# weentiaan/Video-latent-diffusion-panoptic-segmentation

Hardware: NVIDIA B200
Metric: panoptic frames/sec (DDIM-50, 384x1248 KITTI) (higher is better)
Workload: dtype bf16

## Files before the change

video_latent_diffusion_panoptic_segmentation_b200/csrc/gemm_tc.cu:

```cuda
#include <stdlib.h>
#include <string.h>

#include "gemm_tc_kernel.cuh"

namespace ldm_gemm {
#define LDM_GEMM_DECLARE(NAME)                                                                                      \
  cudaError_t NAME(bool pair, int grid, int smem_bytes, cudaStream_t stream, const CUtensorMap& tmA1,               \
                   const CUtensorMap& tmA2, const CUtensorMap& tmB, const CUtensorMap& tmO, const CUtensorMap& tmR, \
                   const CUtensorMap& tmE, const GemmParams& p);
LDM_GEMM_DECLARE(launch_gemm_staged)
LDM_GEMM_DECLARE(launch_gemm_geglu)
LDM_GEMM_DECLARE(launch_gemm_qkv)
LDM_GEMM_DECLARE(launch_gemm_direct)
LDM_GEMM_DECLARE(launch_gemm_convt)
LDM_GEMM_DECLARE(launch_gemm_split)
LDM_GEMM_DECLARE(launch_gemm_geglu_ln)
LDM_GEMM_DECLARE(launch_gemm_qkv_ln)
}

namespace {

using namespace ldm;
using namespace ldm_gemm;

void pick_box(int H, int W, int taps, int* bw_out, int* bh_out) {
  (void)taps;
  if (H == 1) {
    *bw_out = W < 128 ? W : 128;
    *bh_out = 1;
    return;
  }
  long best_tiles = -1;
  int best_bw = 1, best_bh = 1;
  for (int bw = 1; bw <= 128 && bw <= W; ++bw) {
    int bh = 128 / bw;
    if (bh > H) bh = H;
    if (bh < 1) continue;
    const long tiles = (long)((W + bw - 1) / bw) * ((H + bh - 1) / bh);
    if (best_tiles < 0 || tiles < best_tiles || (tiles == best_tiles && bw > best_bw)) {
      best_tiles = tiles;
      best_bw = bw;
      best_bh = bh;
    }
  }
  *bw_out = best_bw;
  *bh_out = best_bh;
}

int pick_block_n(int N, long m_tiles, long kblocks, int sms, bool pair, int taps, double* cost_out, int max_split = 1,
                 long ws_floats = 0, int* split_out = nullptr) {
  static const int cands[] = {256, 224, 192, 160, 128, 96};
  static const double mma_single[] = {167, 158, 151, 141, 111, 106};
  static const double mma_pair[] = {160, 149, 136, 124, 99, 92};
  static const int splits[] = {1, 2, 3, 4, 5, 6, 8, 10, 12, 16};
  int best = 256, best_s = 256, best_split = 1;
  double best_cost = -1.0, best_cost_s = -1.0;
  const long m_units = pair ? (m_tiles + 1) / 2 : m_tiles;
  const long m_alloc = pair ? 2 * m_units : m_units;
  const long workers = pair ? sms / 2 : sms;
  for (int i = 0; i < 6; ++i) {
    const int c = cands[i];
    if (c == 224 && taps != 9) continue;
    const long n_tiles = (N + c - 1) / c;
    for (int si = 0; si < 10; ++si) {
      const int sp = splits[si];
      if (sp > max_split) break;
      if (sp > 1) {
        if (kblocks / sp < (pair ? 24 : 8)) break;
        if ((long)sp * m_alloc * n_tiles * c * 128 > ws_floats) break;
      }
      const long waves = (m_units * n_tiles * sp + workers - 1) / workers;
      const double item = (double)((kblocks + sp - 1) / sp) * 4.0 * (pair ? mma_pair[i] : mma_single[i]) +
                          (pair ? 3300.0 + 11.0 * c : 1000.0 + 17.0 * c) + (sp > 1 ? 8.0 * c : 0.0);
      double cost = (double)waves * item;
      if (sp > 1) cost += 6000.0 + (double)sp * m_alloc * n_tiles * c * 128.0 * 4.0 / 2000.0;
      if (sp == 1) {
        if (best_cost < 0 || cost < best_cost * 0.999) {
          best_cost = cost;
          best = c;
        }
      } else if (best_cost_s < 0 || cost < best_cost_s * 0.999) {
        best_cost_s = cost;
        best_s = c;
        best_split = sp;
      }
    }
  }
  if (best_cost_s > 0 && best_cost_s < 0.88 * best_cost) {
    best_cost = best_cost_s;
    best = best_s;
  } else {
    best_split = 1;
  }
  if (cost_out) *cost_out = best_cost;
  if (split_out) *split_out = best_split;
  return best;
}

int debug_flags() {
  using ldm_host::diag_env_has;
  int v = 0;
  if (diag_env_has("LDM_GEMM_DEBUG", "notma")) v |= kDbgNoTma;
  if (diag_env_has("LDM_GEMM_DEBUG", "nomma")) v |= kDbgNoMma;
  if (diag_env_has("LDM_GEMM_DEBUG", "nowait")) v |= kDbgNoWait | kDbgNoTma;
  if (diag_env_has("LDM_GEMM_DEBUG", "nofence")) v |= kDbgNoFence;
  if (diag_env_has("LDM_GEMM_DEBUG", "keepcommit")) v |= kDbgKeepCommit;
  return v;
}

int resmma_max_kblocks() { return ldm_host::diag_env("LDM_GEMM_RESMMA", 1 << 30); }

bool staged_enabled() { return ldm_host::diag_env("LDM_GEMM_STAGED", 1) != 0; }

bool splitk_enabled() { return ldm_host::diag_env("LDM_GEMM_SPLITK", 1) != 0; }

thread_local int g_last_cfg[3] = {0, 0, 1};

constexpr size_t kSplitCounterBytes = 0;

struct FixupParams {
  const float* ws;
  long long slice_stride;
  int split, tiles_x, tiles_y, bw, bh, W, H, m_tiles, n_tiles, block_n, N, silu;
  const float* bias;
  const float* rowbias;
  const __nv_bfloat16* residual;
  __nv_bfloat16* out;
};

__global__ void __launch_bounds__(256) splitk_fixup_kernel(const FixupParams p) {
  __shared__ float tile[kBlockM][17];
  pdl_launch_dependents();
  pdl_wait();
  const int cb = blockIdx.x, n_tile = blockIdx.y, m_tile = blockIdx.z;
  const int warp = threadIdx.x >> 5, lane = threadIdx.x & 31;
  const long long tile_off = ((long long)m_tile * p.n_tiles + n_tile) * (long long)(p.block_n * kBlockM);
  {
    float a[8];
#pragma unroll
    for (int k = 0; k < 8; ++k) a[k] = 0.f;
    const float* src = p.ws + tile_off + (long long)(cb * 16 + warp * 2) * kBlockM + lane;
    for (int s0 = 0; s0 < p.split; s0 += 4) {
      float v[4][8];
#pragma unroll
      for (int q = 0; q < 4; ++q)
#pragma unroll
        for (int k = 0; k < 8; ++k)
          v[q][k] = s0 + q < p.split ? __ldcg(src + (long long)(s0 + q) * p.slice_stride + (k >> 2) * kBlockM + (k & 3) * 32) : 0.f;
#pragma unroll
      for (int q = 0; q < 4; ++q)
#pragma unroll
        for (int k = 0; k < 8; ++k) a[k] += v[q][k];
    }
#pragma unroll
    for (int k = 0; k < 8; ++k) tile[(k & 3) * 32 + lane][warp * 2 + (k >> 2)] = a[k];
  }
  __syncthreads();
  const int r = threadIdx.x >> 1, vec = threadIdx.x & 1;
  const int tiles_per_img = p.tiles_x * p.tiles_y;
  const int b = m_tile / tiles_per_img;
  const int rem = m_tile - b * tiles_per_img;
  const int ty = rem / p.tiles_x, tx = rem - ty * p.tiles_x;
  const int ly = r / p.bw, lx = r - ly * p.bw;
  const int y = ty * p.bh + ly, x = tx * p.bw + lx;
  const int n = n_tile * p.block_n + cb * 16 + vec * 8;
  if (r >= p.bw * p.bh || y >= p.H || x >= p.W || n >= p.N) return;
  const long long grow = ((long long)b * p.H + y) * p.W + x;
  float f[8];
#pragma unroll
  for (int j = 0; j < 8; ++j) f[j] = tile[r][vec * 8 + j];
  if (p.bias) {
    const float4 b0 = __ldg(reinterpret_cast<const float4*>(p.bias + n)), b1 = __ldg(reinterpret_cast<const float4*>(p.bias + n + 4));
    f[0] += b0.x; f[1] += b0.y; f[2] += b0.z; f[3] += b0.w; f[4] += b1.x; f[5] += b1.y; f[6] += b1.z; f[7] += b1.w;
  }
  if (p.rowbias) {
    const float* rb = p.rowbias + (long long)b * p.N + n;
    const float4 b0 = __ldg(reinterpret_cast<const float4*>(rb)), b1 = __ldg(reinterpret_cast<const float4*>(rb + 4));
    f[0] += b0.x; f[1] += b0.y; f[2] += b0.z; f[3] += b0.w; f[4] += b1.x; f[5] += b1.y; f[6] += b1.z; f[7] += b1.w;
  }
  if (p.residual) {
    const uint4 u = ld_nc_v4(p.residual + grow * p.N + n);
    const float2 a0 = unpack_bf16(u.x), a1 = unpack_bf16(u.y), a2 = unpack_bf16(u.z), a3 = unpack_bf16(u.w);
    f[0] += a0.x; f[1] += a0.y; f[2] += a1.x; f[3] += a1.y; f[4] += a2.x; f[5] += a2.y; f[6] += a3.x; f[7] += a3.y;
  }
  if (p.silu) {
#pragma unroll
    for (int j = 0; j < 8; ++j) f[j] = silu_f(f[j]);
  }
  store_bf16x8(p.out + grow * p.N + n, f);
// ... 325 lines not shown
```

video_latent_diffusion_panoptic_segmentation_b200/csrc/gemm_tc_kernel.cuh:

```cuda
#pragma once
#include "common.cuh"
#include "host_util.h"

namespace ldm_gemm {

using namespace ldm;

constexpr int kBlockM = 128;
constexpr int kBlockK = 64;
constexpr int kABytes = kBlockM * kBlockK * 2;
constexpr int kMaxStages = 8;
constexpr int kEpiWarps = 8;
constexpr int kThreads = 64 + 32 * kEpiWarps;
constexpr int kSmemBudget = 227 * 1024;
constexpr int kEpiStageBytes = 2 * 16384 + 1280;
constexpr int kStagedStore = 1 << 20;
constexpr int kQkvStaged = 1 << 21;
constexpr int kDbgNoTma = 1 << 29;
constexpr int kDbgNoMma = 1 << 30;
constexpr int kDbgNoFence = 1 << 27;
constexpr int kDbgKeepCommit = 1 << 26;
constexpr int kDbgNoWait = 1 << 28;

struct GemmParams {
  int tiles_x, tiles_y, B, bw, bh, W, H;
  int m_tiles, n_tiles, block_n;
  int N, taps, kblocks1, kblocks, ktap;
  int stages, stage_bytes;
  int res_kblocks;
  int flags;
  const float* bias;
  const float* rowbias;
  const __nv_bfloat16* residual;
  void* out;
  __nv_bfloat16* q;
  __nv_bfloat16* k;
  __nv_bfloat16* vt;
  const float* ln_gamma;
  const float* ln_beta;
  float ln_eps;
  int heads, head_dim, dpad, seq, seq_pad, vt_rows;
  int qkv_part0;
  unsigned long long magic_seq, magic_c, magic_d;
  int a_stride;
  int a_pad;
  int up2_ntiles;
  int up2_cout;
  int n_store;
  long long img_px;
  float* row_stats;
  const float* ln_stats;
  const float* ln_colsum;
  int ln_parts;
  long long rows_total;
  float ln_invc, ln_fold_eps;
  int split_k;
  float* ws;
  long long ws_slice_stride;
};

__device__ __forceinline__ void store_bf16x8(__nv_bfloat16* dst, const float* v) {
  uint4 u;
  u.x = pack_bf16(v[0], v[1]);
  u.y = pack_bf16(v[2], v[3]);
  u.z = pack_bf16(v[4], v[5]);
  u.w = pack_bf16(v[6], v[7]);
  *reinterpret_cast<uint4*>(dst) = u;
}

enum { kEpiStaged = 0, kEpiGeglu = 1, kEpiQkv = 2, kEpiDirect = 3, kEpiConvT = 4, kEpiSplit = 5, kEpiGegluLn = 6, kEpiQkvLn = 7 };

template <bool kPair, int kEpiT>
__global__ void __launch_bounds__(kThreads, 1)
gemm_tc_kernel(const __grid_constant__ CUtensorMap tmA1, const __grid_constant__ CUtensorMap tmA2,
               const __grid_constant__ CUtensorMap tmB, const __grid_constant__ CUtensorMap tmO,
               const __grid_constant__ CUtensorMap tmR, const __grid_constant__ CUtensorMap tmE, const GemmParams p) {
  constexpr bool kLn = kEpiT == kEpiGegluLn || kEpiT == kEpiQkvLn;
  constexpr int kEpi = kEpiT == kEpiGegluLn ? (int)kEpiGeglu : kEpiT == kEpiQkvLn ? (int)kEpiQkv : kEpiT;
  extern __shared__ __align__(1024) uint8_t smem_raw[];
  uint8_t* smem = smem_raw + ((1024u - (smem_u32(smem_raw) & 1023u)) & 1023u);
  uint8_t* epi_smem = smem + p.stages * p.stage_bytes;
  uint64_t* full_bar = reinterpret_cast<uint64_t*>(epi_smem + kEpiStageBytes);
  uint64_t* empty_bar = full_bar + kMaxStages;
  uint64_t* tfull_bar = empty_bar + kMaxStages;
  uint64_t* tempty_bar = tfull_bar + 2;
  uint32_t* tmem_slot = reinterpret_cast<uint32_t*>(tempty_bar + 2);

  const int warp = __shfl_sync(0xffffffffu, (int)(threadIdx.x >> 5), 0);
  const int lane = threadIdx.x & 31;
  const uint32_t rank = kPair ? cluster_ctarank() : 0u;
  const int worker = kPair ? (int)(blockIdx.x >> 1) : (int)blockIdx.x;
  const int num_workers = kPair ? (int)(gridDim.x >> 1) : (int)gridDim.x;

  if (warp == 0 && lane == 0) {
    tma_prefetch_desc(&tmA1);
    tma_prefetch_desc(&tmA2);
    tma_prefetch_desc(&tmB);
    tma_prefetch_desc(&tmO);
    for (int i = 0; i < p.stages; ++i) {
      mbar_init(&full_bar[i], 1);
      mbar_init(&empty_bar[i], 1);
    }
    for (int i = 0; i < 2; ++i) {
      mbar_init(&tfull_bar[i], 1);
      mbar_init(&tempty_bar[i], (kPair ? 2 : 1) * kEpiWarps);
    }
    mbar_fence_init();
  }
  if (warp == 1) {
    if (kPair) {
      tmem_alloc_pair(tmem_slot, 512);
      tmem_relinquish_pair();
    } else {
      tmem_alloc(tmem_slot, 512);
      tmem_relinquish();
    }
  }
  tc_fence_before();
  if (kPair) cluster_sync_all(); else __syncthreads();
  tc_fence_after();
  const uint32_t tmem_base = *tmem_slot;
  pdl_launch_dependents();
  pdl_wait();

  const int m_units = kPair ? (p.m_tiles + 1) / 2 : p.m_tiles;
  const int num_tiles = m_units * p.n_tiles;
  constexpr bool kSplit = kEpi == kEpiSplit;
  const int split = kSplit ? p.split_k : 1;
  const int num_items = num_tiles * split;
  const int kmain = p.taps * p.kblocks;
  const int tiles_per_img = p.tiles_x * p.tiles_y;
  const uint32_t a_bytes = (uint32_t)(p.bw * p.bh) * (kBlockK * 2);
  const int b_rows = kPair ? p.block_n / 2 : p.block_n;
  const uint32_t b_bytes = (uint32_t)b_rows * (kBlockK * 2);

  if (warp == 0) {
    {
      int stage = 0;
      uint32_t phase = 0;
      for (int item = worker; item < num_items; item += num_workers) {
        const int tile = kSplit ? item / split : item;
        const int slice = kSplit ? item - tile * split : 0;
        const int k_lo = kSplit ? (int)((long long)kmain * slice / split) : 0;
        const int k_hi = kSplit ? (int)((long long)kmain * (slice + 1) / split) : kmain;
        const int n_tile = tile / m_units;
        const int m_unit = tile - n_tile * m_units;
        const int m_tile = kPair ? 2 * m_unit + (int)rank : m_unit;
        const int b = m_tile / tiles_per_img;
        const int rem = m_tile - b * tiles_per_img;
        const int ty = rem / p.tiles_x;
        const int tx = rem - ty * p.tiles_x;
        const int x0 = tx * p.bw, y0 = ty * p.bh;
        const int n0 = n_tile * p.block_n + (int)rank * b_rows;
        int tap = k_lo / p.kblocks, kb = k_lo - tap * p.kblocks;
        const int cls = p.up2_ntiles > 0 ? n_tile / p.up2_ntiles : 0;
        const int ax0 = x0 * p.a_stride, ay0 = y0 * p.a_stride;
        for (int ki = k_lo; ki < k_hi; ++ki) {
          const int dy = (p.taps == 9) ? tap / 3 - p.a_pad : (p.taps == 4) ? (tap >> 1) - 1 + (cls >> 1) : 0;
          const int dx = (p.taps == 9) ? tap % 3 - p.a_pad : (p.taps == 4) ? (tap & 1) - 1 + (cls & 1) : 0;
          {
            if (p.flags & kDbgNoWait) continue;
            mbar_wait(&empty_bar[stage], phase ^ 1);
            uint8_t* sa = smem + stage * p.stage_bytes;
            uint8_t* sb = sa + kABytes;
            const CUtensorMap* tmA = (kb < p.kblocks1) ? &tmA1 : &tmA2;
            const int kc = (kb < p.kblocks1 ? kb : kb - p.kblocks1) * kBlockK;
            if (!elect_one()) {
            } else if (p.flags & kDbgNoTma) {
              if (rank == 0) mbar_arrive(&full_bar[stage]);
            } else if (kPair) {
              if (rank == 0) mbar_arrive_expect_tx(&full_bar[stage], 2 * (a_bytes + b_bytes));
              tma_load_4d_pair(sa, tmA, &full_bar[stage], kc, ax0 + dx, ay0 + dy, b);
              tma_load_2d_pair(sb, &tmB, &full_bar[stage], tap * p.ktap + kb * kBlockK, n0);
            } else {
              mbar_arrive_expect_tx(&full_bar[stage], a_bytes + b_bytes);
              tma_load_4d(sa, tmA, &full_bar[stage], kc, ax0 + dx, ay0 + dy, b);
              tma_load_2d(sb, &tmB, &full_bar[stage], tap * p.ktap + kb * kBlockK, n0);
            }
            if (++stage == p.stages) {
              stage = 0;
              phase ^= 1;
            }
          }
          if (++kb == p.kblocks) {
            kb = 0;
            ++tap;
          }
        }
        const int nres = (slice == split - 1) ? p.res_kblocks : 0;
        for (int j = 0; j < nres; ++j) {
          mbar_wait(&empty_bar[stage], phase ^ 1);
          uint8_t* sa = smem + stage * p.stage_bytes;
          uint8_t* sb = sa + kABytes;
          if (elect_one()) {
            if (kPair) {
              if (rank == 0) mbar_arrive_expect_tx(&full_bar[stage], 2 * (a_bytes + b_bytes));
              tma_load_4d_pair(sa, &tmR, &full_bar[stage], n_tile * p.block_n + j * kBlockK, x0, y0, b);
              tma_load_2d_pair(sb, &tmE, &full_bar[stage], j * kBlockK, (int)rank * b_rows);
            } else {
              mbar_arrive_expect_tx(&full_bar[stage], a_bytes + b_bytes);
              tma_load_4d(sa, &tmR, &full_bar[stage], n_tile * p.block_n + j * kBlockK, x0, y0, b);
              tma_load_2d(sb, &tmE, &full_bar[stage], j * kBlockK, 0);
            }
          }
          if (++stage == p.stages) {
            stage = 0;
            phase ^= 1;
          }
        }
      }
    }
    __syncwarp();
  } else if (warp == 1) {
    if (rank == 0) {
      const uint32_t idesc = umma_idesc_bf16(kPair ? 256 : kBlockM, (uint32_t)p.block_n);
      int stage = 0;
      uint32_t phase = 0;
      int as = 0;
      uint32_t aphase = 0;
      for (int item = worker; item < num_items; item += num_workers) {
        int ksteps = kmain + p.res_kblocks;
        if (kSplit) {
          const int slice = item % split;
          ksteps = (int)((long long)kmain * (slice + 1) / split) - (int)((long long)kmain * slice / split) +
                   (slice == split - 1 ? p.res_kblocks : 0);
        }
        mbar_wait(&tempty_bar[as], aphase ^ 1);
        tc_fence_after();
        const uint32_t d_tmem = tmem_base + (uint32_t)as * 256u;
        for (int ks = 0; ks < ksteps; ++ks) {
          if (!(p.flags & kDbgNoWait)) {
            mbar_wait(&full_bar[stage], phase);
            if (!(p.flags & kDbgNoFence)) tc_fence_after();
          }
          const uint32_t sa = smem_u32(smem + stage * p.stage_bytes);
          const uint64_t da = umma_desc_k_sw128(sa);
          const uint64_t db = umma_desc_k_sw128(sa + kABytes);
          if (elect_one()) {
#pragma unroll
            for (int k = 0; k < kBlockK / 16; ++k) {
              if (p.flags & kDbgNoMma) break;
              const uint32_t dt = d_tmem;
              if (kPair)
                umma_bf16_pair(dt, da + (uint64_t)(2 * k), db + (uint64_t)(2 * k), idesc, (ks | k) != 0);
              else
                umma_bf16(dt, da + (uint64_t)(2 * k), db + (uint64_t)(2 * k), idesc, (ks | k) != 0);
            }
            if ((p.flags & kDbgNoWait) && !(p.flags & kDbgKeepCommit)) {
            } else if (kPair) umma_commit_pair(&empty_bar[stage]); else umma_commit(&empty_bar[stage]);
          }
          __syncwarp();
          if (++stage == p.stages) {
            stage = 0;
            phase ^= 1;
          }
        }
        if (elect_one()) {
          if (kPair) umma_commit_pair(&tfull_bar[as]); else umma_commit(&tfull_bar[as]);
        }
        __syncwarp();
        if (++as == 2) {
          as = 0;
          aphase ^= 1;
        }
      }
    }
    __syncwarp();
  } else {
    const int quad = warp & 3;
    const int half = (warp - 2) >> 2;
    const int r = quad * 32 + lane;
    constexpr bool geglu = kEpi == kEpiGeglu;
    constexpr bool staged = kEpi == kEpiStaged || kEpi == kEpiGeglu;
    const bool plain = kEpi == kEpiStaged || (kEpi == kEpiDirect && !(p.flags & LDM_GEMM_GEGLU));
    const bool epi_leader = threadIdx.x == 64;
    int sb = 0;
    int as = 0;
    uint32_t aphase = 0;
    constexpr int kLnPre = 20;
    [[maybe_unused]] float2 ln_pre[kLnPre];
    [[maybe_unused]] auto ln_issue = [&](int item2) {
      const int tile2 = kSplit ? item2 / split : item2;
      const int n_tile2 = tile2 / m_units;
      const int m_unit2 = tile2 - n_tile2 * m_units;
      const int m_tile2 = kPair ? 2 * m_unit2 + (int)rank : m_unit2;
      const int b2 = m_tile2 / tiles_per_img;
      const int rem2 = m_tile2 - b2 * tiles_per_img;
      const int ty2 = rem2 / p.tiles_x;
      const int tx2 = rem2 - ty2 * p.tiles_x;
      const int ly2 = r / p.bw, lx2 = r - ly2 * p.bw;
      const int y2 = ty2 * p.bh + ly2, x2 = tx2 * p.bw + lx2;
      const bool valid2 = (m_tile2 < p.m_tiles) && (r < p.bw * p.bh) && (y2 < p.H) && (x2 < p.W);
      const float2* sp = reinterpret_cast<const float2*>(p.ln_stats) + (((long long)b2 * p.H + y2) * p.W + x2);
#pragma unroll
      for (int j = 0; j < kLnPre; ++j)
        ln_pre[j] = (valid2 && j < p.ln_parts) ? __ldg(sp + (long long)j * p.rows_total) : make_float2(0.f, 0.f);
    };
    if constexpr (kLn) {
      if (worker < num_items) ln_issue(worker);
    }
    for (int item = worker; item < num_items; item += num_workers) {
      const int tile = kSplit ? item / split : item;
      const int slice = kSplit ? item - tile * split : 0;
      const int n_tile = tile / m_units;
      const int m_unit = tile - n_tile * m_units;
      const int m_tile = kPair ? 2 * m_unit + (int)rank : m_unit;
      const int b = m_tile / tiles_per_img;
      const int rem = m_tile - b * tiles_per_img;
      const int ty = rem / p.tiles_x;
      const int tx = rem - ty * p.tiles_x;
      const int ly = r / p.bw, lx = r - ly * p.bw;
      const int y = ty * p.bh + ly, x = tx * p.bw + lx;
      const bool valid = (m_tile < p.m_tiles) && (r < p.bw * p.bh) && (y < p.H) && (x < p.W);
      const long long grow = ((long long)b * p.H + y) * p.W + x;
      const int n0 = n_tile * p.block_n;
      int qkv_bi = 0, qkv_s = 0;
      const bool qkv_vec = kEpi == kEpiQkv && (p.seq % 8 == 0) && p.bh == 1 && p.bw == kBlockM;
      if (kEpi == kEpiQkv) {
        qkv_bi = (int)(((unsigned long long)grow * p.magic_seq) >> 40);
        qkv_s = (int)(grow - (long long)qkv_bi * p.seq);
      }

      float ln_a = 1.f, ln_c = 0.f;
      constexpr bool ln_fold = kLn;
      if constexpr (ln_fold) {
        float su = 0.f, sq = 0.f;
#pragma unroll
        for (int j = 0; j < kLnPre; ++j) {
          su += ln_pre[j].x;
          sq += ln_pre[j].y;
        }
        if (valid) {
          const float2* sp = reinterpret_cast<const float2*>(p.ln_stats) + grow;
          for (int i = kLnPre; i < p.ln_parts; i += 10) {
            float2 t[10];
#pragma unroll
            for (int j = 0; j < 10; ++j)
              t[j] = i + j < p.ln_parts ? __ldg(sp + (long long)(i + j) * p.rows_total) : make_float2(0.f, 0.f);
#pragma unroll
            for (int j = 0; j < 10; ++j) {
              su += t[j].x;
              sq += t[j].y;
            }
          }
        }
        const float mean = su * p.ln_invc;
        ln_a = rsqrtf(fmaxf(fmaf(-mean, mean, sq * p.ln_invc), 0.f) + p.ln_fold_eps);
        ln_c = -mean * ln_a;
        if (item + num_workers < num_items) ln_issue(item + num_workers);
      }
      const bool ln_smem = kEpi == kEpiQkv && ln_fold && p.block_n <= 160;
      float* sLn = reinterpret_cast<float*>(epi_smem + 2 * 16384);
      if (ln_smem) {
        named_bar_sync(1, 32 * kEpiWarps);
        const int t = threadIdx.x - 64;
        if (t < p.block_n) {
          const int n = n0 + t;
          sLn[t] = (p.bias && n < p.N) ? __ldg(p.bias + n) : 0.f;
          sLn[160 + t] = n < p.N ? __ldg(p.ln_colsum + n) : 0.f;
        }
        named_bar_sync(1, 32 * kEpiWarps);
      }
      uint4 rs[4][4];
      const bool use_res = !kSplit && plain && p.residual != nullptr && valid && p.res_kblocks == 0;
      if (use_res) {
        const __nv_bfloat16* rrow = p.residual + grow * p.N + n0;
#pragma unroll
        for (int ci = 0; ci < 4; ++ci) {
          const int c = staged ? (ci * 64 < p.block_n ? min(ci * 64, p.block_n - 64) + half * 32 : p.block_n)
                               : (2 * ci + half) * 32;
#pragma unroll
          for (int g = 0; g < 4; ++g)
            if (c < p.block_n && n0 + c + g * 8 < p.N) rs[ci][g] = ld_nc_v4(rrow + c + g * 8);
        }
      }

      constexpr bool tile_bias = staged && !kSplit && !kLn;
      if constexpr (tile_bias) {
        float* sbias = reinterpret_cast<float*>(epi_smem + 2 * 16384);
        const int t = threadIdx.x - 64;
        if (t < p.block_n) {
          const int n = n0 + t;
          float bv = 0.f;
          if (n < p.N) {
            if (p.bias) bv = __ldg(p.bias + n);
            if (p.rowbias) bv += __ldg(p.rowbias + (long long)b * p.N + n);
          }
          sbias[t] = bv;
        }
      }
      mbar_wait(&tfull_bar[as], aphase);
      tc_fence_after();
      const uint32_t t_addr = tmem_base + ((uint32_t)(quad * 32) << 16) + (uint32_t)as * 256u;

      if constexpr (kSplit) {
        const long long tile_off = ((long long)m_tile * p.n_tiles + n_tile) * (long long)(p.block_n * kBlockM);
        float* wdst = p.ws + (long long)slice * p.ws_slice_stride + tile_off + r;
        for (int c = half * 32; c < p.block_n; c += 64) {
          uint32_t v[32];
          tmem_ld32(t_addr + c, v);
          tmem_ld_wait();
#pragma unroll
          for (int j = 0; j < 32; ++j) wdst[(c + j) * kBlockM] = __uint_as_float(v[j]);
        }
      }

      if constexpr (kSplit) {
      } else if constexpr (kEpi == kEpiConvT) {
        if (half == 0) {
        const int cout = p.block_n;
        float mean = 0.f;
        for (int c = 0; c < cout; c += 32) {
          uint32_t v[32];
          tmem_ld32(t_addr + c, v);
          tmem_ld_wait();
#pragma unroll
          for (int j = 0; j < 32; ++j) mean += __uint_as_float(v[j]) + __ldg(&p.bias[n0 + c + j]);
        }
        mean /= (float)cout;
        float var = 0.f;
        for (int c = 0; c < cout; c += 32) {
          uint32_t v[32];
          tmem_ld32(t_addr + c, v);
          tmem_ld_wait();
#pragma unroll
          for (int j = 0; j < 32; ++j) {
            const float d = __uint_as_float(v[j]) + __ldg(&p.bias[n0 + c + j]) - mean;
            var += d * d;
          }
        }
        const float rstd = 1.0f / sqrtf(var / (float)cout + p.ln_eps);
        const int sub = n_tile;
        const long long orow = ((long long)b * (2 * p.H) + (2 * y + (sub >> 1))) * (2 * p.W) + (2 * x + (sub & 1));
        __nv_bfloat16* dst = reinterpret_cast<__nv_bfloat16*>(p.out) + orow * cout;
        for (int c = 0; c < cout; c += 32) {
          uint32_t v[32];
          tmem_ld32(t_addr + c, v);
          tmem_ld_wait();
          if (valid) {
#pragma unroll
            for (int g = 0; g < 4; ++g) {
              float o[8];
#pragma unroll
              for (int j = 0; j < 8; ++j) {
                const int cc = c + g * 8 + j;
                const float xn = (__uint_as_float(v[g * 8 + j]) + __ldg(&p.bias[n0 + cc]) - mean) * rstd;
                o[j] = silu_f(__ldg(&p.ln_gamma[cc]) * xn + __ldg(&p.ln_beta[cc]));
              }
              store_bf16x8(dst + c + g * 8, o);
            }
          }
        }
        }
      } else if constexpr (staged) {
        const int acc_w = geglu ? 128 : 64;
#pragma unroll
        for (int ob = 0; ob < 4; ++ob) {
          if (ob * acc_w >= p.block_n) break;
          const int c0 = min(ob * acc_w, p.block_n - acc_w);
          uint8_t* sbuf = epi_smem + sb * 16384;
          float* sbias = reinterpret_cast<float*>(epi_smem + 2 * 16384);
          float* sgsum = sbias + 128;
          if (epi_leader) bulk_wait_read1();
          if constexpr (!tile_bias) {
            const int t = threadIdx.x - 64;
            if (t < acc_w) {
              const int n = n0 + c0 + t;
              float bv = 0.f;
              if (n < p.N) {
                if (p.bias) bv = __ldg(p.bias + n);
                if (p.rowbias) bv += __ldg(p.rowbias + (long long)b * p.N + n);
              }
              sbias[t] = bv;
              if (ln_fold) sgsum[t] = n < p.N ? __ldg(p.ln_colsum + n) : 0.f;
            }
          }
          named_bar_sync(1, 32 * kEpiWarps);
          uint8_t* rowp = sbuf + r * 128;
#pragma unroll
          for (int cq = 0; cq < 2; ++cq) {
            if (!geglu && cq == 1) break;
            const int cc = geglu ? half * 64 + cq * 32 : half * 32;
            const int c = c0 + cc;
            uint32_t v[32];
            tmem_ld32(t_addr + c, v);
            const int nc = n0 + c;
            float f[32];
            {
              const float4* bp = reinterpret_cast<const float4*>(sbias + (tile_bias ? c : cc));
              if (ln_fold) {
                tmem_ld_wait();
                const float4* gp = reinterpret_cast<const float4*>(sgsum + cc);
#pragma unroll
                for (int g = 0; g < 8; ++g) {
                  const float4 bv = bp[g], gv = gp[g];
                  f[g * 4] = fmaf(ln_a, __uint_as_float(v[g * 4]), fmaf(ln_c, gv.x, bv.x));
                  f[g * 4 + 1] = fmaf(ln_a, __uint_as_float(v[g * 4 + 1]), fmaf(ln_c, gv.y, bv.y));
                  f[g * 4 + 2] = fmaf(ln_a, __uint_as_float(v[g * 4 + 2]), fmaf(ln_c, gv.z, bv.z));
                  f[g * 4 + 3] = fmaf(ln_a, __uint_as_float(v[g * 4 + 3]), fmaf(ln_c, gv.w, bv.w));
                }
              } else {
                float4 bv[8];
#pragma unroll
                for (int g = 0; g < 8; ++g) bv[g] = bp[g];
                tmem_ld_wait();
#pragma unroll
                for (int g = 0; g < 8; ++g) {
                  f[g * 4] = __uint_as_float(v[g * 4]) + bv[g].x;
                  f[g * 4 + 1] = __uint_as_float(v[g * 4 + 1]) + bv[g].y;
                  f[g * 4 + 2] = __uint_as_float(v[g * 4 + 2]) + bv[g].z;
                  f[g * 4 + 3] = __uint_as_float(v[g * 4 + 3]) + bv[g].w;
                }
              }
            }
            if (geglu) {
              float o[16];
#pragma unroll
              for (int j = 0; j < 16; ++j) o[j] = f[j] * gelu_erf_fast(f[16 + j]);
#pragma unroll
              for (int g = 0; g < 2; ++g) {
                uint4 u;
                u.x = pack_bf16(o[g * 8 + 0], o[g * 8 + 1]); u.y = pack_bf16(o[g * 8 + 2], o[g * 8 + 3]);
                u.z = pack_bf16(o[g * 8 + 4], o[g * 8 + 5]); u.w = pack_bf16(o[g * 8 + 6], o[g * 8 + 7]);
                *reinterpret_cast<uint4*>(rowp + ((((cc >> 5) * 2 + g) ^ (r & 7)) << 4)) = u;
              }
            } else {
              if (use_res) {
#pragma unroll
                for (int g = 0; g < 4; ++g) {
                  if (nc + g * 8 >= p.N) break;
                  const uint4 u = rs[ob][g];
                  const float2 a0 = unpack_bf16(u.x), a1 = unpack_bf16(u.y), a2 = unpack_bf16(u.z), a3 = unpack_bf16(u.w);
                  f[g * 8 + 0] += a0.x; f[g * 8 + 1] += a0.y; f[g * 8 + 2] += a1.x; f[g * 8 + 3] += a1.y;
                  f[g * 8 + 4] += a2.x; f[g * 8 + 5] += a2.y; f[g * 8 + 6] += a3.x; f[g * 8 + 7] += a3.y;
                }
              }
              if (p.flags & LDM_GEMM_SILU) {
#pragma unroll
                for (int j = 0; j < 32; ++j) f[j] = silu_f(f[j]);
              }
              float st_s = 0.f, st_q = 0.f;
#pragma unroll
              for (int g = 0; g < 4; ++g) {
                uint4 u;
                u.x = pack_bf16(f[g * 8 + 0], f[g * 8 + 1]); u.y = pack_bf16(f[g * 8 + 2], f[g * 8 + 3]);
                u.z = pack_bf16(f[g * 8 + 4], f[g * 8 + 5]); u.w = pack_bf16(f[g * 8 + 6], f[g * 8 + 7]);
                *reinterpret_cast<uint4*>(rowp + (((half * 4 + g) ^ (r & 7)) << 4)) = u;
                if (kEpi == kEpiStaged && p.row_stats) {
                  const float2 a0 = unpack_bf16(u.x), a1 = unpack_bf16(u.y), a2 = unpack_bf16(u.z), a3 = unpack_bf16(u.w);
                  st_s += ((a0.x + a0.y) + (a1.x + a1.y)) + ((a2.x + a2.y) + (a3.x + a3.y));
                  st_q = fmaf(a0.x, a0.x, st_q); st_q = fmaf(a0.y, a0.y, st_q); st_q = fmaf(a1.x, a1.x, st_q);
                  st_q = fmaf(a1.y, a1.y, st_q); st_q = fmaf(a2.x, a2.x, st_q); st_q = fmaf(a2.y, a2.y, st_q);
                  st_q = fmaf(a3.x, a3.x, st_q); st_q = fmaf(a3.y, a3.y, st_q);
                }
              }
              if (kEpi == kEpiStaged && p.row_stats && valid && nc < p.N)
                *reinterpret_cast<float2*>(p.row_stats + ((long long)(nc >> 5) * p.rows_total + grow) * 2) =
                    make_float2(st_s, st_q);
            }
          }
          fence_proxy_async_smem();
          named_bar_sync(1, 32 * kEpiWarps);
          if (epi_leader) {
            if (p.up2_ntiles > 0) {
              const int cls = n_tile / p.up2_ntiles;
              tma_store_4d(&tmO, sbuf, n0 + c0 - cls * p.up2_cout, 2 * tx * p.bw + (cls & 1), 2 * ty * p.bh + (cls >> 1), b);
            } else {
              const int ncol = geglu ? (n0 + c0) / 2 : n0 + c0;
              tma_store_4d(&tmO, sbuf, ncol, tx * p.bw, ty * p.bh, b);
            }
            bulk_commit();
          }
          sb ^= 1;
        }
      } else {
        bool qkv_done = false;
        if constexpr (kEpi == kEpiQkv) {
          const int C = p.heads * p.head_dim;
          const int part_in = n0 / C;
          const int which_t = part_in + p.qkv_part0;
          const long long grow0 = (long long)m_tile * kBlockM;
          const int bi0 = (int)(((unsigned long long)grow0 * p.magic_seq) >> 40);
          const int s0 = (int)(grow0 - (long long)bi0 * p.seq);
          const int nimg = (int)(((long long)p.W * p.H * p.B) / p.seq);
          if ((p.flags & kQkvStaged) && which_t < 2 && (s0 + kBlockM <= p.seq || bi0 + 1 >= nimg)) {
            const int head0 = (n0 - part_in * C) / p.head_dim;
            const int heads_in_tile = p.block_n / p.head_dim;
            const int blocks_per_head = p.dpad >> 6;
            for (int hd = 0; hd < heads_in_tile; ++hd) {
              for (int kb = 0; kb < blocks_per_head; ++kb) {
                uint8_t* sbuf = epi_smem + sb * 16384;
                if (epi_leader) bulk_wait_read1();
                named_bar_sync(1, 32 * kEpiWarps);
                const int cbase = hd * p.head_dim + kb * 64 + half * 32;
                int ng = ((hd + 1) * p.head_dim - cbase) >> 3;
                ng = ng < 0 ? 0 : (ng > 4 ? 4 : ng);
                uint32_t v[32];
#pragma unroll
                for (int g = 0; g < 4; ++g)
                  if (g < ng) tmem_ld8(t_addr + cbase + g * 8, v + g * 8);
                tmem_ld_wait();
                if (ln_fold) {
#pragma unroll
                  for (int g = 0; g < 4; ++g)
                    if (g < ng) {
                      const int cl = cbase + g * 8;
                      float4 g0, g1, b0, b1;
                      if (ln_smem) {
                        b0 = *reinterpret_cast<const float4*>(sLn + cl);
                        b1 = *reinterpret_cast<const float4*>(sLn + cl + 4);
                        g0 = *reinterpret_cast<const float4*>(sLn + 160 + cl);
                        g1 = *reinterpret_cast<const float4*>(sLn + 160 + cl + 4);
                      } else {
                        const int n = n0 + cl;
                        g0 = __ldg(reinterpret_cast<const float4*>(p.ln_colsum + n));
                        g1 = __ldg(reinterpret_cast<const float4*>(p.ln_colsum + n + 4));
                        b0 = make_float4(0.f, 0.f, 0.f, 0.f), b1 = b0;
                        if (p.bias) {
                          b0 = __ldg(reinterpret_cast<const float4*>(p.bias + n));
                          b1 = __ldg(reinterpret_cast<const float4*>(p.bias + n + 4));
                        }
                      }
                      const float gv[8] = {g0.x, g0.y, g0.z, g0.w, g1.x, g1.y, g1.z, g1.w};
                      const float bv[8] = {b0.x, b0.y, b0.z, b0.w, b1.x, b1.y, b1.z, b1.w};
#pragma unroll
                      for (int j = 0; j < 8; ++j)
                        v[g * 8 + j] = __float_as_uint(fmaf(ln_a, __uint_as_float(v[g * 8 + j]), fmaf(ln_c, gv[j], bv[j])));
                    }
                }
                uint8_t* rowp = sbuf + r * 128;
#pragma unroll
                for (int g = 0; g < 4; ++g) {
                  uint4 u = make_uint4(0, 0, 0, 0);
                  if (g < ng) {
                    u.x = pack_bf16(__uint_as_float(v[g * 8 + 0]), __uint_as_float(v[g * 8 + 1]));
                    u.y = pack_bf16(__uint_as_float(v[g * 8 + 2]), __uint_as_float(v[g * 8 + 3]));
                    u.z = pack_bf16(__uint_as_float(v[g * 8 + 4]), __uint_as_float(v[g * 8 + 5]));
                    u.w = pack_bf16(__uint_as_float(v[g * 8 + 6]), __uint_as_float(v[g * 8 + 7]));
                  }
                  *reinterpret_cast<uint4*>(rowp + (((half * 4 + g) ^ (r & 7)) << 4)) = u;
                }
                fence_proxy_async_smem();
                named_bar_sync(1, 32 * kEpiWarps);
                if (epi_leader) {
                  if (which_t == 0) tma_store_4d(&tmO, sbuf, kb * 64, s0, head0 + hd, bi0);
                  else tma_store_4d(&tmR, sbuf, kb * 64, s0, head0 + hd, bi0);
                  bulk_commit();
                }
                sb ^= 1;
              }
            }
            qkv_done = true;
          }
          if ((p.flags & kQkvStaged) && !qkv_done) {
            if (epi_leader) bulk_wait_read0();
            named_bar_sync(1, 32 * kEpiWarps);
          }
        }
#pragma unroll
        for (int ci = 0; ci < 4; ++ci) {
          if (qkv_done) break;
          const int c = (2 * ci + half) * 32;
          if (c >= p.block_n) break;
          uint32_t v[32];
          tmem_ld32(t_addr + c, v);
          tmem_ld_wait();
          if (!valid && kEpi != kEpiQkv) continue;
          const int nc = n0 + c;
          if (nc >= p.N) continue;
          float f[32];
#pragma unroll
          for (int j = 0; j < 32; ++j) f[j] = __uint_as_float(v[j]);
          if (ln_smem) {
            const float4* bp = reinterpret_cast<const float4*>(sLn + c);
            const float4* gp = reinterpret_cast<const float4*>(sLn + 160 + c);
#pragma unroll
            for (int g = 0; g < 8; ++g)
              if (nc + g * 4 < p.N) {
                const float4 gv = gp[g], bv = bp[g];
                f[g * 4] = fmaf(ln_a, f[g * 4], fmaf(ln_c, gv.x, bv.x));
                f[g * 4 + 1] = fmaf(ln_a, f[g * 4 + 1], fmaf(ln_c, gv.y, bv.y));
                f[g * 4 + 2] = fmaf(ln_a, f[g * 4 + 2], fmaf(ln_c, gv.z, bv.z));
                f[g * 4 + 3] = fmaf(ln_a, f[g * 4 + 3], fmaf(ln_c, gv.w, bv.w));
              }
          } else if (ln_fold) {
            const float4* gp = reinterpret_cast<const float4*>(p.ln_colsum + nc);
#pragma unroll
            for (int g = 0; g < 8; ++g)
              if (nc + g * 4 < p.N) {
                const float4 gv = __ldg(gp + g);
                f[g * 4] = fmaf(ln_a, f[g * 4], ln_c * gv.x); f[g * 4 + 1] = fmaf(ln_a, f[g * 4 + 1], ln_c * gv.y);
                f[g * 4 + 2] = fmaf(ln_a, f[g * 4 + 2], ln_c * gv.z); f[g * 4 + 3] = fmaf(ln_a, f[g * 4 + 3], ln_c * gv.w);
              }
          }
          if (p.bias && !ln_smem) {
            const float4* bp = reinterpret_cast<const float4*>(p.bias + nc);
#pragma unroll
            for (int g = 0; g < 8; ++g)
              if (nc + g * 4 < p.N) {
                const float4 bv = __ldg(bp + g);
                f[g * 4] += bv.x; f[g * 4 + 1] += bv.y; f[g * 4 + 2] += bv.z; f[g * 4 + 3] += bv.w;
              }
          }
          if (p.rowbias) {
            const float4* bp = reinterpret_cast<const float4*>(p.rowbias + (long long)b * p.N + nc);
#pragma unroll
            for (int g = 0; g < 8; ++g)
              if (nc + g * 4 < p.N) {
                const float4 bv = __ldg(bp + g);
                f[g * 4] += bv.x; f[g * 4 + 1] += bv.y; f[g * 4 + 2] += bv.z; f[g * 4 + 3] += bv.w;
              }
          }
          if (p.flags & LDM_GEMM_GEGLU) {
            float o[16];
#pragma unroll
            for (int j = 0; j < 16; ++j) o[j] = f[j] * gelu_erf_fast(f[16 + j]);
            __nv_bfloat16* dst = reinterpret_cast<__nv_bfloat16*>(p.out) + grow * (p.N / 2) + nc / 2;
            store_bf16x8(dst, o);
            store_bf16x8(dst + 8, o + 8);
            continue;
          }
          if constexpr (kEpi == kEpiQkv) {
            const int C = p.heads * p.head_dim;
#pragma unroll
            for (int g = 0; g < 4; ++g) {
              const int n = nc + g * 8;
              if (n >= p.N) break;
              const int part = (int)(((unsigned long long)(unsigned)n * p.magic_c) >> 40);
              const int cc = n - part * C;
              const int which = part + p.qkv_part0;
              const int head = (int)(((unsigned long long)(unsigned)cc * p.magic_d) >> 40);
              const int e = cc - head * p.head_dim;
              const long long bh = (long long)qkv_bi * p.heads + head;
              if (which < 2) {
                if (valid) {
                  __nv_bfloat16* dst = (which == 0 ? p.q : p.k) + (bh * p.seq + qkv_s) * p.dpad + e;
                  store_bf16x8(dst, f + g * 8);
                }
              } else if (qkv_vec) {
                __nv_bfloat16* sT = reinterpret_cast<__nv_bfloat16*>(epi_smem) + (warp - 2) * 256;
#pragma unroll
                for (int j = 0; j < 8; ++j) sT[j * 32 + lane] = __float2bfloat16_rn(f[g * 8 + j]);
                __syncwarp();
                const int cch = lane >> 2, tq = lane & 3;
                const uint4 u = *reinterpret_cast<const uint4*>(sT + cch * 32 + tq * 8);
                __syncwarp();
                const int g_bi = __shfl_sync(0xffffffffu, qkv_bi, tq * 8), g_s = __shfl_sync(0xffffffffu, qkv_s, tq * 8);
                const int g_ok = __shfl_sync(0xffffffffu, (int)valid, tq * 8);
                if (g_ok) {
                  __nv_bfloat16* dst =
                      p.vt + (((long long)g_bi * p.heads + head) * p.vt_rows + e + cch) * p.seq_pad + g_s;
                  *reinterpret_cast<uint4*>(dst) = u;
                }
              } else if (valid) {
                __nv_bfloat16* dst = p.vt + (bh * p.vt_rows + e) * p.seq_pad + qkv_s;
#pragma unroll
                for (int j = 0; j < 8; ++j) dst[(long long)j * p.seq_pad] = __float2bfloat16_rn(f[g * 8 + j]);
              }
            }
            continue;
          }
          if (use_res) {
#pragma unroll
            for (int g = 0; g < 4; ++g) {
              if (nc + g * 8 >= p.N) break;
              const uint4 u = rs[ci][g];
              const float2 a0 = unpack_bf16(u.x), a1 = unpack_bf16(u.y), a2 = unpack_bf16(u.z), a3 = unpack_bf16(u.w);
              f[g * 8 + 0] += a0.x; f[g * 8 + 1] += a0.y; f[g * 8 + 2] += a1.x; f[g * 8 + 3] += a1.y;
              f[g * 8 + 4] += a2.x; f[g * 8 + 5] += a2.y; f[g * 8 + 6] += a3.x; f[g * 8 + 7] += a3.y;
            }
          }
          if (p.flags & LDM_GEMM_SILU) {
#pragma unroll
            for (int j = 0; j < 32; ++j) f[j] = silu_f(f[j]);
          }
          if (p.flags & LDM_GEMM_OUT_NCHW_F32) {
            const long long bi = grow / p.img_px, pix = grow - bi * p.img_px;
            float* dst = reinterpret_cast<float*>(p.out) + (bi * p.n_store) * p.img_px + pix;
#pragma unroll
            for (int j = 0; j < 32; ++j)
              if (nc + j < p.n_store) dst[(long long)(nc + j) * p.img_px] = f[j];
            continue;
          }
          if (p.flags & LDM_GEMM_OUT_F32) {
            float* dst = reinterpret_cast<float*>(p.out) + grow * p.N + nc;
#pragma unroll
            for (int g = 0; g < 8; ++g) {
              if (nc + g * 4 >= p.N) break;
              *reinterpret_cast<float4*>(dst + g * 4) = make_float4(f[g * 4], f[g * 4 + 1], f[g * 4 + 2], f[g * 4 + 3]);
            }
          } else {
            __nv_bfloat16* dst = reinterpret_cast<__nv_bfloat16*>(p.out) + grow * p.N + nc;
#pragma unroll
            for (int g = 0; g < 4; ++g) {
              if (nc + g * 8 >= p.N) break;
              store_bf16x8(dst + g * 8, f + g * 8);
            }
          }
        }
      }
      tc_fence_before();
      __syncwarp();
      if (lane == 0) {
        if (kPair) mbar_arrive_cluster(&tempty_bar[as], 0); else mbar_arrive(&tempty_bar[as]);
      }
      if (++as == 2) {
        as = 0;
        aphase ^= 1;
      }
    }
  }

  if (threadIdx.x == 64) bulk_wait_all();
  tc_fence_before();
  if (kPair) cluster_sync_all(); else __syncthreads();
  if (warp == 1) {
    tc_fence_after();
    if (kPair) tmem_dealloc_pair(tmem_base, 512); else tmem_dealloc(tmem_base, 512);
  }
}

}
```

Baseline: 9.276.

## Add dedicated TMA store warp with mbarrier handoff and prefetched tile bias

Adds an eleventh warp that issues the epilogue TMA stores, waits on bulk-read completion, and recycles the two smem staging buffers through new stage_full/stage_free mbarriers. This takes the leader thread's bulk_wait and the named barrier syncs off the epilogue warps. The store warp also prefetches per-tile bias into registers and publishes it through a bias mbarrier. The epilogue double-buffers TMEM loads, interleaves residual loads, and releases the accumulator earlier. The cost is an extra warp, more barrier state, and a new 'noepi' debug flag.

```diff
diff --git a/video_latent_diffusion_panoptic_segmentation_b200/csrc/gemm_tc.cu b/video_latent_diffusion_panoptic_segmentation_b200/csrc/gemm_tc.cu
--- a/video_latent_diffusion_panoptic_segmentation_b200/csrc/gemm_tc.cu
+++ b/video_latent_diffusion_panoptic_segmentation_b200/csrc/gemm_tc.cu
@@ -105,6 +105,7 @@
   if (diag_env_has("LDM_GEMM_DEBUG", "nowait")) v |= kDbgNoWait | kDbgNoTma;
   if (diag_env_has("LDM_GEMM_DEBUG", "nofence")) v |= kDbgNoFence;
   if (diag_env_has("LDM_GEMM_DEBUG", "keepcommit")) v |= kDbgKeepCommit;
+  if (diag_env_has("LDM_GEMM_DEBUG", "noepi")) v |= kDbgNoEpi;
   return v;
 }
 
diff --git a/video_latent_diffusion_panoptic_segmentation_b200/csrc/gemm_tc_kernel.cuh b/video_latent_diffusion_panoptic_segmentation_b200/csrc/gemm_tc_kernel.cuh
--- a/video_latent_diffusion_panoptic_segmentation_b200/csrc/gemm_tc_kernel.cuh
+++ b/video_latent_diffusion_panoptic_segmentation_b200/csrc/gemm_tc_kernel.cuh
@@ -11,7 +11,8 @@
 constexpr int kABytes = kBlockM * kBlockK * 2;
 constexpr int kMaxStages = 8;
 constexpr int kEpiWarps = 8;
-constexpr int kThreads = 64 + 32 * kEpiWarps;
+constexpr int kStoreWarp = 2 + kEpiWarps;
+constexpr int kThreads = 32 * (kStoreWarp + 1);
 constexpr int kSmemBudget = 227 * 1024;
 constexpr int kEpiStageBytes = 2 * 16384 + 1280;
 constexpr int kStagedStore = 1 << 20;
@@ -21,6 +22,7 @@
 constexpr int kDbgNoFence = 1 << 27;
 constexpr int kDbgKeepCommit = 1 << 26;
 constexpr int kDbgNoWait = 1 << 28;
+constexpr int kDbgNoEpi = 1 << 25;
 
 struct GemmParams {
   int tiles_x, tiles_y, B, bw, bh, W, H;
@@ -84,7 +86,11 @@
   uint64_t* empty_bar = full_bar + kMaxStages;
   uint64_t* tfull_bar = empty_bar + kMaxStages;
   uint64_t* tempty_bar = tfull_bar + 2;
-  uint32_t* tmem_slot = reinterpret_cast<uint32_t*>(tempty_bar + 2);
+  uint64_t* stage_full = tempty_bar + 2;
+  uint64_t* stage_free = stage_full + 2;
+  uint64_t* bias_full = stage_free + 2;
+  uint32_t* tmem_slot = reinterpret_cast<uint32_t*>(bias_full + 1);
+  int* stage_desc = reinterpret_cast<int*>(bias_full + 2);
 
   const int warp = __shfl_sync(0xffffffffu, (int)(threadIdx.x >> 5), 0);
   const int lane = threadIdx.x & 31;
@@ -104,7 +110,10 @@
     for (int i = 0; i < 2; ++i) {
       mbar_init(&tfull_bar[i], 1);
       mbar_init(&tempty_bar[i], (kPair ? 2 : 1) * kEpiWarps);
+      mbar_init(&stage_full[i], kEpiWarps);
+      mbar_init(&stage_free[i], 1);
     }
+    mbar_init(bias_full, 1);
     mbar_fence_init();
   }
   if (warp == 1) {
@@ -133,6 +142,10 @@
   const uint32_t a_bytes = (uint32_t)(p.bw * p.bh) * (kBlockK * 2);
   const int b_rows = kPair ? p.block_n / 2 : p.block_n;
   const uint32_t b_bytes = (uint32_t)b_rows * (kBlockK * 2);
+  constexpr bool staged = kEpi == kEpiStaged || kEpi == kEpiGeglu;
+  const bool store_warp = !(p.flags & kDbgNoEpi) && (staged || (kEpi == kEpiQkv && (p.flags & kQkvStaged)));
+  constexpr bool tile_bias = staged && !kLn;
+  float* sbias = reinterpret_cast<float*>(epi_smem + 2 * 16384);
 
   if (warp == 0) {
     {
@@ -266,17 +279,96 @@
       }
     }
     __syncwarp();
+  } else if (warp == kStoreWarp) {
+    if (store_warp) {
+      float bias_r[8];
+      auto bias_load = [&](int item2) {
+        const int n_tile2 = item2 / m_units;
+        const int m_unit2 = item2 - n_tile2 * m_units;
+        const int b2 = (kPair ? 2 * m_unit2 + (int)rank : m_unit2) / tiles_per_img;
+#pragma unroll
+        for (int j = 0; j < 8; ++j) {
+          const int t = lane + 32 * j, n = n_tile2 * p.block_n + t;
+          float bv = 0.f;
+          if (t < p.block_n && n < p.N) {
+            if (p.bias) bv = __ldg(p.bias + n);
+            if (p.rowbias) bv += __ldg(p.rowbias + (long long)b2 * p.N + n);
+          }
+          bias_r[j] = bv;
+        }
+      };
+      auto bias_publish = [&]() {
+#pragma unroll
+        for (int j = 0; j < 8; ++j)
+          if (lane + 32 * j < p.block_n) sbias[lane + 32 * j] = bias_r[j];
+        __syncwarp();
+        if (lane == 0) mbar_arrive(bias_full);
+      };
+      if (tile_bias && worker < num_items) {
+        bias_load(worker);
+        bias_publish();
+      }
+      int sb = 0;
+      uint32_t sphase = 0;
+      for (int item = worker; item < num_items; item += num_workers) {
+        const bool more = item + num_workers < num_items;
+        if (tile_bias && more) bias_load(item + num_workers);
+        bool last = false;
+        while (!last) {
+          mbar_wait(&stage_full[sb], sphase);
+          const int* d = stage_desc + sb * 6;
+          const int map = d[4];
+          last = d[5] != 0;
+          if (lane == 0 && map != 0) {
+            tma_store_4d(map == 1 ? &tmO : &tmR, epi_smem + sb * 16384, d[0], d[1], d[2], d[3]);
+            bulk_commit();
+          }
+          if (tile_bias && last && more) bias_publish();
+          __syncwarp();
+          if (lane == 0) {
+            if (map != 0) bulk_wait_read0();
+            mbar_arrive(&stage_free[sb]);
+          }
+          if (++sb == 2) {
+            sb = 0;
+            sphase ^= 1;
+          }
+        }
+      }
+      if (lane == 0) bulk_wait_all();
+    }
+    __syncwarp();
   } else {
     const int quad = warp & 3;
     const int half = (warp - 2) >> 2;
     const int r = quad * 32 + lane;
     constexpr bool geglu = kEpi == kEpiGeglu;
-    constexpr bool staged = kEpi == kEpiStaged || kEpi == kEpiGeglu;
     const bool plain = kEpi == kEpiStaged || (kEpi == kEpiDirect && !(p.flags & LDM_GEMM_GEGLU));
-    const bool epi_leader = threadIdx.x == 64;
-    int sb = 0;
-    int as = 0;
-    uint32_t aphase = 0;
+    uint32_t fills = 0;
+    uint32_t tiles = 0;
+    auto release_acc = [&]() {
+      tc_fence_before();
+      __syncwarp();
+      if (lane == 0) {
+        if (kPair) mbar_arrive_cluster(&tempty_bar[tiles & 1], 0); else mbar_arrive(&tempty_bar[tiles & 1]);
+      }
+    };
+    auto stage_commit = [&](int map, int c0, int c1, int c2, int c3, bool last) {
+      fence_proxy_async_smem();
+      __syncwarp();
+      if (lane == 0) {
+        if (warp == 2) {
+          int* d = stage_desc + (fills & 1) * 6;
+          d[0] = c0; d[1] = c1; d[2] = c2; d[3] = c3; d[4] = map; d[5] = last ? 1 : 0;
+        }
+        mbar_arrive(&stage_full[fills & 1]);
+      }
+      ++fills;
+    };
+    auto stage_acquire = [&]() {
+      mbar_wait(&stage_free[fills & 1], ((fills >> 1) & 1) ^ 1);
+      return epi_smem + (fills & 1) * 16384;
+    };
     constexpr int kLnPre = 20;
     [[maybe_unused]] float2 ln_pre[kLnPre];
     [[maybe_unused]] auto ln_issue = [&](int item2) {
@@ -300,6 +392,13 @@
       if (worker < num_items) ln_issue(worker);
     }
     for (int item = worker; item < num_items; item += num_workers) {
+      if (p.flags & kDbgNoEpi) {
+        mbar_wait(&tfull_bar[tiles & 1], (tiles >> 1) & 1);
+        tc_fence_after();
+        release_acc();
+        ++tiles;
+        continue;
+      }
       const int tile = kSplit ? item / split : item;
       const int slice = kSplit ? item - tile * split : 0;
       const int n_tile = tile / m_units;
@@ -363,35 +462,24 @@
       }
       uint4 rs[4][4];
       const bool use_res = !kSplit && plain && p.residual != nullptr && valid && p.res_kblocks == 0;
+      const __nv_bfloat16* rrow = p.residual + grow * p.N + n0;
+      auto res_load = [&](int ci) {
+        const int c = staged ? (ci * 64 < p.block_n ? min(ci * 64, p.block_n - 64) + half * 32 : p.block_n)
+                             : (2 * ci + half) * 32;
+#pragma unroll
+        for (int g = 0; g < 4; ++g)
+          if (c < p.block_n && n0 + c + g * 8 < p.N) rs[ci][g] = ld_nc_v4(rrow + c + g * 8);
+      };
       if (use_res) {
-        const __nv_bfloat16* rrow = p.residual + grow * p.N + n0;
-#pragma unroll
-        for (int ci = 0; ci < 4; ++ci) {
-          const int c = staged ? (ci * 64 < p.block_n ? min(ci * 64, p.block_n - 64) + half * 32 : p.block_n)
-                               : (2 * ci + half) * 32;
-#pragma unroll
-          for (int g = 0; g < 4; ++g)
-            if (c < p.block_n && n0 + c + g * 8 < p.N) rs[ci][g] = ld_nc_v4(rrow + c + g * 8);
-        }
-      }
-
-      constexpr bool tile_bias = staged && !kSplit && !kLn;
-      if constexpr (tile_bias) {
-        float* sbias = reinterpret_cast<float*>(epi_smem + 2 * 16384);
-        const int t = threadIdx.x - 64;
-        if (t < p.block_n) {
-          const int n = n0 + t;
-          float bv = 0.f;
-          if (n < p.N) {
-            if (p.bias) bv = __ldg(p.bias + n);
-            if (p.rowbias) bv += __ldg(p.rowbias + (long long)b * p.N + n);
-          }
-          sbias[t] = bv;
-        }
-      }
-      mbar_wait(&tfull_bar[as], aphase);
+#pragma unroll
+        for (int ci = 0; ci < (staged ? 1 : 4); ++ci) res_load(ci);
+      }
+
+      mbar_wait(&tfull_bar[tiles & 1], (tiles >> 1) & 1);
       tc_fence_after();
-      const uint32_t t_addr = tmem_base + ((uint32_t)(quad * 32) << 16) + (uint32_t)as * 256u;
+      bool qkv_done = false;
+      if constexpr (tile_bias) mbar_wait(bias_full, tiles & 1);
+      const uint32_t t_addr = tmem_base + ((uint32_t)(quad * 32) << 16) + (tiles & 1) * 256u;
 
       if constexpr (kSplit) {
         const long long tile_off = ((long long)m_tile * p.n_tiles + n_tile) * (long long)(p.block_n * kBlockM);
@@ -454,15 +542,23 @@
         }
       } else if constexpr (staged) {
         const int acc_w = geglu ? 128 : 64;
+        const int nchunks = (geglu ? 2 : 1) * ((p.block_n + acc_w - 1) / acc_w);
+        auto chunk_col = [&](int i) {
+          const int ob = geglu ? i >> 1 : i;
+          return min(ob * acc_w, p.block_n - acc_w) + (geglu ? half * 64 + (i & 1) * 32 : half * 32);
+        };
+        uint32_t v2[2][32];
+        if (geglu) tmem_ld32(t_addr + chunk_col(0), v2[0]);
 #pragma unroll
         for (int ob = 0; ob < 4; ++ob) {
           if (ob * acc_w >= p.block_n) break;
           const int c0 = min(ob * acc_w, p.block_n - acc_w);
-          uint8_t* sbuf = epi_smem + sb * 16384;
-          float* sbias = reinterpret_cast<float*>(epi_smem + 2 * 16384);
+          const bool last_block = (ob + 1) * acc_w >= p.block_n;
+          if (!geglu && use_res && ob < 3) res_load(ob + 1);
+          uint8_t* sbuf = stage_acquire();
           float* sgsum = sbias + 128;
-          if (epi_leader) bulk_wait_read1();
           if constexpr (!tile_bias) {
+            named_bar_sync(1, 32 * kEpiWarps);
             const int t = threadIdx.x - 64;
             if (t < acc_w) {
               const int n = n0 + c0 + t;
@@ -474,22 +570,28 @@
               sbias[t] = bv;
               if (ln_fold) sgsum[t] = n < p.N ? __ldg(p.ln_colsum + n) : 0.f;
             }
-          }
-          named_bar_sync(1, 32 * kEpiWarps);
+            named_bar_sync(1, 32 * kEpiWarps);
+          }
           uint8_t* rowp = sbuf + r * 128;
 #pragma unroll
           for (int cq = 0; cq < 2; ++cq) {
             if (!geglu && cq == 1) break;
             const int cc = geglu ? half * 64 + cq * 32 : half * 32;
             const int c = c0 + cc;
-            uint32_t v[32];
-            tmem_ld32(t_addr + c, v);
+            const int ci = geglu ? 2 * ob + cq : ob;
+            if (!geglu) tmem_ld32(t_addr + c, v2[ci & 1]);
+            tmem_ld_wait();
+            if (ci + 1 < nchunks) {
+              if (geglu) tmem_ld32(t_addr + chunk_col(ci + 1), v2[(ci + 1) & 1]);
+            } else {
+              release_acc();
+            }
+            const uint32_t* v = v2[ci & 1];
             const int nc = n0 + c;
             float f[32];
             {
               const float4* bp = reinterpret_cast<const float4*>(sbias + (tile_bias ? c : cc));
               if (ln_fold) {
-                tmem_ld_wait();
                 const float4* gp = reinterpret_cast<const float4*>(sgsum + cc);
 #pragma unroll
                 for (int g = 0; g < 8; ++g) {
@@ -500,16 +602,13 @@
                   f[g * 4 + 3] = fmaf(ln_a, __uint_as_float(v[g * 4 + 3]), fmaf(ln_c, gv.w, bv.w));
                 }
               } else {
-                float4 bv[8];
-#pragma unroll
-                for (int g = 0; g < 8; ++g) bv[g] = bp[g];
-                tmem_ld_wait();
 #pragma unroll
                 for (int g = 0; g < 8; ++g) {
-                  f[g * 4] = __uint_as_float(v[g * 4]) + bv[g].x;
-                  f[g * 4 + 1] = __uint_as_float(v[g * 4 + 1]) + bv[g].y;
-                  f[g * 4 + 2] = __uint_as_float(v[g * 4 + 2]) + bv[g].z;
-                  f[g * 4 + 3] = __uint_as_float(v[g * 4 + 3]) + bv[g].w;
+                  const float4 bv = bp[g];
+                  f[g * 4] = __uint_as_float(v[g * 4]) + bv.x;
+                  f[g * 4 + 1] = __uint_as_float(v[g * 4 + 1]) + bv.y;
+                  f[g * 4 + 2] = __uint_as_float(v[g * 4 + 2]) + bv.z;
+                  f[g * 4 + 3] = __uint_as_float(v[g * 4 + 3]) + bv.w;
                 }
               }
             }
@@ -559,22 +658,14 @@
                     make_float2(st_s, st_q);
             }
           }
-          fence_proxy_async_smem();
-          named_bar_sync(1, 32 * kEpiWarps);
-          if (epi_leader) {
-            if (p.up2_ntiles > 0) {
-              const int cls = n_tile / p.up2_ntiles;
-              tma_store_4d(&tmO, sbuf, n0 + c0 - cls * p.up2_cout, 2 * tx * p.bw + (cls & 1), 2 * ty * p.bh + (cls >> 1), b);
-            } else {
-              const int ncol = geglu ? (n0 + c0) / 2 : n0 + c0;
-              tma_store_4d(&tmO, sbuf, ncol, tx * p.bw, ty * p.bh, b);
-            }
-            bulk_commit();
-          }
-          sb ^= 1;
+          if (p.up2_ntiles > 0) {
+            const int cls = n_tile / p.up2_ntiles;
+            stage_commit(1, n0 + c0 - cls * p.up2_cout, 2 * tx * p.bw + (cls & 1), 2 * ty * p.bh + (cls >> 1), b, last_block);
+          } else {
+            stage_commit(1, geglu ? (n0 + c0) / 2 : n0 + c0, tx * p.bw, ty * p.bh, b, last_block);
+          }
         }
       } else {
-        bool qkv_done = false;
         if constexpr (kEpi == kEpiQkv) {
           const int C = p.heads * p.head_dim;
           const int part_in = n0 / C;
@@ -589,9 +680,8 @@
             const int blocks_per_head = p.dpad >> 6;
             for (int hd = 0; hd < heads_in_tile; ++hd) {
               for (int kb = 0; kb < blocks_per_head; ++kb) {
-                uint8_t* sbuf = epi_smem + sb * 16384;
-                if (epi_leader) bulk_wait_read1();
-                named_bar_sync(1, 32 * kEpiWarps);
+                const bool last_block = hd == heads_in_tile - 1 && kb == blocks_per_head - 1;
+                uint8_t* sbuf = stage_acquire();
                 const int cbase = hd * p.head_dim + kb * 64 + half * 32;
                 int ng = ((hd + 1) * p.head_dim - cbase) >> 3;
                 ng = ng < 0 ? 0 : (ng > 4 ? 4 : ng);
@@ -640,21 +730,14 @@
                   }
                   *reinterpret_cast<uint4*>(rowp + (((half * 4 + g) ^ (r & 7)) << 4)) = u;
                 }
-                fence_proxy_async_smem();
-                named_bar_sync(1, 32 * kEpiWarps);
-                if (epi_leader) {
-                  if (which_t == 0) tma_store_4d(&tmO, sbuf, kb * 64, s0, head0 + hd, bi0);
-                  else tma_store_4d(&tmR, sbuf, kb * 64, s0, head0 + hd, bi0);
-                  bulk_commit();
-                }
-                sb ^= 1;
+                if (last_block) release_acc();
+                stage_commit(which_t == 0 ? 1 : 2, kb * 64, s0, head0 + hd, bi0, last_block);
               }
             }
             qkv_done = true;
           }
           if ((p.flags & kQkvStaged) && !qkv_done) {
-            if (epi_leader) bulk_wait_read0();
-            named_bar_sync(1, 32 * kEpiWarps);
+            stage_acquire();
           }
         }
 #pragma unroll
@@ -738,7 +821,7 @@
                   store_bf16x8(dst, f + g * 8);
                 }
               } else if (qkv_vec) {
-                __nv_bfloat16* sT = reinterpret_cast<__nv_bfloat16*>(epi_smem) + (warp - 2) * 256;
+                __nv_bfloat16* sT = reinterpret_cast<__nv_bfloat16*>(epi_smem + (fills & 1) * 16384) + (warp - 2) * 256;
 #pragma unroll
                 for (int j = 0; j < 8; ++j) sT[j * 32 + lane] = __float2bfloat16_rn(f[g * 8 + j]);
                 __syncwarp();
@@ -798,20 +881,13 @@
             }
           }
         }
-      }
-      tc_fence_before();
-      __syncwarp();
-      if (lane == 0) {
-        if (kPair) mbar_arrive_cluster(&tempty_bar[as], 0); else mbar_arrive(&tempty_bar[as]);
-      }
-      if (++as == 2) {
-        as = 0;
-        aphase ^= 1;
-      }
+        if (kEpi == kEpiQkv && (p.flags & kQkvStaged) && !qkv_done) stage_commit(0, 0, 0, 0, 0, true);
+      }
+      if (!staged && !qkv_done) release_acc();
+      ++tiles;
     }
   }
 
-  if (threadIdx.x == 64) bulk_wait_all();
   tc_fence_before();
   if (kPair) cluster_sync_all(); else __syncthreads();
   if (warp == 1) {
```

New measurement: 9.188 (median of 6 runs). No clear change (-0.9%).
